# hyye/lio-mapping

Hardware: AMD Instinct MI355X
Metric: sliding-window solves/sec, 64-line 130k-pt scans, window=15 (opt_window=5) (higher is better)
Workload: dtype f64 (solve) / f32 (features); 1 GPU; HDL-64E outdoor_test_config_64, S_outdoor ray-cast scans, window_size=15 opt_window_size=5, one SolveOptimization per step, clouds resident in HBM; n_lidar_residuals=78236, local_map_points=76752, surf_stack_points=19386, parallelism=1 window

## Files before the change

lio-mapping_amd/csrc/capi.hip:

```cpp
#include <cstring>
#include <new>

#include "../../include/lio_c.h"
#include "../../include/lio_test_hooks.h"
#include "est_batch.h"
#include "seg_sort.h"
#include "estimator.h"
#include "rccl_comm.h"
#include "host_init.h"
#include "kf_batch.h"
#include <mutex>
#include <thread>
#include <atomic>

#include "mapping.h"
#include "odometry.h"
#include "pointproc.h"

using namespace lio;

struct lio_pim { std::shared_ptr<Preintegration> p; };
struct lio_est { std::unique_ptr<Estimator> e; EstConfig cfg; std::unique_ptr<MappingDev> map; lio_map_config map_cfg; std::unique_ptr<EstimatorBatch> solo; bool adopted = false; struct lio_est_batch *owner = nullptr; };
struct lio_est_batch {
  std::unique_ptr<EstimatorBatch> b, b2;
// ... 433 lines not shown
  if (!T || !out || (!corner && nc) || (!surf && ns) || (!full && nf)) return 0;
  float *o = out;
  *o++ = T->p[0]; *o++ = T->p[1]; *o++ = T->p[2]; *o++ = 0.f;
  *o++ = T->q[0]; *o++ = T->q[1]; *o++ = T->q[2]; *o++ = T->q[3];
  *o++ = float(nc); *o++ = float(ns); *o++ = float(nf); *o++ = T->q[3];
  const float *src[3] = {corner, surf, full};
  const size_t cnt[3] = {nc, ns, nf};
  for (int k = 0; k < 3; ++k) { if (cnt[k]) std::memcpy(o, src[k], cnt[k] * 4 * sizeof(float)); o += 4 * cnt[k]; }
  return size_t(o - out) / 4;
}
int lio_compact_decode(const float *d, size_t n, lio_transform_f *T, size_t *nc, size_t *ns, size_t *nf) {
  if (!d || !nc || !ns || !nf || n < 4) return LIO_ERR_ARG;
  const float lim = float(n);
  for (int k = 8; k <= 10; ++k)
    if (!(d[k] >= 0.0f && d[k] <= lim)) return LIO_ERR_ARG;
  const unsigned long long c = (unsigned long long)d[8], s = (unsigned long long)d[9], f = (unsigned long long)d[10];
  if (3ull + c + s + f != (unsigned long long)n) return LIO_ERR_ARG;
  if (T) { for (int k = 0; k < 3; ++k) T->p[k] = d[k]; for (int k = 0; k < 4; ++k) T->q[k] = d[4 + k]; }
  *nc = size_t(c); *ns = size_t(s); *nf = size_t(f);
  return LIO_OK;
}

struct Scratch {
  hipStream_t s = nullptr;
  DBuf<float4> a, b, c;
  VoxelGridDev vox;
  KnnGrid grid;
  DBuf<uint8_t> valid;
  DBuf<float4> coef;
  DBuf<float> score, tf;
  DBuf<int32_t> idx;
  DBuf<float> sqd;
  DBuf<float> bounds;
};
static Scratch &scratch() {
  static thread_local Scratch sc;
  if (!sc.s) {
    int nd = 0;
    LIO_HIP(hipGetDeviceCount(&nd));
    if (nd <= 0) throw DeviceError("no HIP device: the product has no CPU path");
    LIO_HIP(hipStreamCreate(&sc.s));
  }
  return sc;
}
static void host_bounds(const float *xyzi, size_t n, float mn[3], float mx[3]) {
  for (int d = 0; d < 3; ++d) { mn[d] = 3.4e38f; mx[d] = -3.4e38f; }
  for (size_t i = 0; i < n; ++i)
    for (int d = 0; d < 3; ++d) { float v = xyzi[4 * i + d]; if (std::isfinite(v)) { mn[d] = std::min(mn[d], v); mx[d] = std::max(mx[d], v); } }
}

int lio_voxel_grid(const float *xyzi, size_t n, float leaf, float *out, size_t *n_out) {
  if ((!xyzi && n) || !out || !n_out || !(leaf > 0)) return LIO_ERR_ARG;
  return guarded([&] {
    Scratch &sc = scratch();
    sc.a.reserve(std::max<size_t>(n, 1));
    if (n) LIO_HIP(hipMemcpyAsync(sc.a.p, xyzi, n * sizeof(float4), hipMemcpyHostToDevice, sc.s));
    size_t m = sc.vox.run(sc.a.p, n, leaf, sc.b, sc.s);
    if (m) LIO_HIP(hipMemcpyAsync(out, sc.b.p, m * sizeof(float4), hipMemcpyDeviceToHost, sc.s));
    LIO_HIP(hipStreamSynchronize(sc.s));
    *n_out = m;
    return LIO_OK;
  });
}

int lio_knn(const float *map, size_t n_map, const float *query, size_t m, int k, float radius_sq, int32_t *idx, float *sqd) {
  if ((!map && n_map) || (!query && m) || !(k == 1 || k == 5) || !idx || !sqd) return LIO_ERR_ARG;
  if (!(radius_sq > 0)) return LIO_ERR_ARG;
  return guarded([&] {
    Scratch &sc = scratch();
    sc.a.reserve(std::max<size_t>(n_map, 1)); sc.b.reserve(std::max<size_t>(m, 1));
    sc.idx.reserve(std::max<size_t>(m * k, 1)); sc.sqd.reserve(std::max<size_t>(m * k, 1));
    if (n_map) LIO_HIP(hipMemcpyAsync(sc.a.p, map, n_map * sizeof(float4), hipMemcpyHostToDevice, sc.s));
    if (m) LIO_HIP(hipMemcpyAsync(sc.b.p, query, m * sizeof(float4), hipMemcpyHostToDevice, sc.s));
    float mn[3], mx[3];
    host_bounds(map, n_map, mn, mx);
    if (n_map == 0) { mn[0] = mn[1] = mn[2] = 0; mx[0] = mx[1] = mx[2] = 0; }
    sc.grid.build(sc.a.p, n_map, mn, mx, std::sqrt(radius_sq) * 1.0001f + 1e-6f, sc.s);
    launch_knn(sc.b.p, int(m), k, radius_sq, sc.grid.sorted(), sc.grid.cells(), sc.grid.desc(), sc.idx.p, sc.sqd.p, sc.s);
    if (m) {
      LIO_HIP(hipMemcpyAsync(idx, sc.idx.p, m * k * sizeof(int32_t), hipMemcpyDeviceToHost, sc.s));
      LIO_HIP(hipMemcpyAsync(sqd, sc.sqd.p, m * k * sizeof(float), hipMemcpyDeviceToHost, sc.s));
    }
    LIO_HIP(hipStreamSynchronize(sc.s));
    return LIO_OK;
  });
}

int lio_calculate_features(const float *map, size_t n_map, const float *stack, size_t m, const lio_transform_f *T, float mm, float mp,
                           uint8_t *valid, float *coeff, float *score) {
  if ((!map && n_map) || (!stack && m) || !T || !valid || !coeff || !score || !(mm > 0)) return LIO_ERR_ARG;
  return guarded([&] {
    Scratch &sc = scratch();
    sc.a.reserve(std::max<size_t>(n_map, 1)); sc.b.reserve(std::max<size_t>(m, 1));
    sc.valid.reserve(std::max<size_t>(m, 1)); sc.coef.reserve(std::max<size_t>(m, 1)); sc.score.reserve(std::max<size_t>(m, 1)); sc.tf.reserve(8);
    if (n_map) LIO_HIP(hipMemcpyAsync(sc.a.p, map, n_map * sizeof(float4), hipMemcpyHostToDevice, sc.s));
    if (m) LIO_HIP(hipMemcpyAsync(sc.b.p, stack, m * sizeof(float4), hipMemcpyHostToDevice, sc.s));
    float tf[8] = {T->q[0], T->q[1], T->q[2], T->q[3], T->p[0], T->p[1], T->p[2], 0.f};
    LIO_HIP(hipMemcpyAsync(sc.tf.p, tf, sizeof(tf), hipMemcpyHostToDevice, sc.s));
    float mn[3], mx[3];
    host_bounds(map, n_map, mn, mx);
    if (n_map == 0) { mn[0] = mn[1] = mn[2] = 0; mx[0] = mx[1] = mx[2] = 0; }
    sc.grid.build(sc.a.p, n_map, mn, mx, std::sqrt(mm) * 1.0001f + 1e-6f, sc.s);
    FeatArgs fa{};
    fa.nframes = 1; fa.max_M = int(m); fa.min_match_sq_dis = mm; fa.min_plane_dis = mp;
    fa.fr[0].stack = sc.b.p; fa.fr[0].M = int(m); fa.fr[0].slot_off = 0; fa.fr[0].tf_index = 0;
    launch_features(fa, sc.tf.p, sc.grid.sorted(), sc.grid.cells(), sc.grid.desc(), sc.valid.p, sc.coef.p, sc.score.p, nullptr, sc.s);
    if (m) {
      LIO_HIP(hipMemcpyAsync(valid, sc.valid.p, m, hipMemcpyDeviceToHost, sc.s));
      LIO_HIP(hipMemcpyAsync(coeff, sc.coef.p, m * sizeof(float4), hipMemcpyDeviceToHost, sc.s));
      LIO_HIP(hipMemcpyAsync(score, sc.score.p, m * sizeof(float), hipMemcpyDeviceToHost, sc.s));
    }
    LIO_HIP(hipStreamSynchronize(sc.s));
    return LIO_OK;
  });
}

lio_pim *lio_pim_create(const double acc0[3], const double gyr0[3], const double ba[3], const double bg[3], double acc_n, double gyr_n,
                        double acc_w, double gyr_w, double g_norm) {
  if (!acc0 || !gyr0 || !ba || !bg) return nullptr;
  PimNoise n; n.acc_n = acc_n; n.gyr_n = gyr_n; n.acc_w = acc_w; n.gyr_w = gyr_w; n.g_norm = g_norm;
  lio_pim *h = new (std::nothrow) lio_pim;
  if (h) h->p = std::make_shared<Preintegration>(v3(acc0), v3(gyr0), v3(ba), v3(bg), n);
  return h;
}
void lio_pim_destroy(lio_pim *h) { delete h; }
int lio_pim_push_back(lio_pim *h, double dt, const double acc[3], const double gyr[3]) {
  if (!h || !acc || !gyr) return LIO_ERR_ARG;
  h->p->push_back(dt, v3(acc), v3(gyr));
  return LIO_OK;
}
int lio_pim_repropagate(lio_pim *h, const double ba[3], const double bg[3]) {
  if (!h || !ba || !bg) return LIO_ERR_ARG;
  h->p->repropagate(v3(ba), v3(bg));
  return LIO_OK;
}
int lio_pim_get(const lio_pim *h, double *sum_dt, double *dp, double *dq, double *dv, double *jac, double *cov) {
  if (!h) return LIO_ERR_ARG;
  const Preintegration &p = *h->p;
  if (sum_dt) *sum_dt = p.sum_dt;
  if (dp) { dp[0] = p.dp.x; dp[1] = p.dp.y; dp[2] = p.dp.z; }
  if (dq) { dq[0] = p.dq.x; dq[1] = p.dq.y; dq[2] = p.dq.z; dq[3] = p.dq.w; }
  if (dv) { dv[0] = p.dv.x; dv[1] = p.dv.y; dv[2] = p.dv.z; }
  if (jac) std::memcpy(jac, p.jac, sizeof(p.jac));
  if (cov) std::memcpy(cov, p.cov, sizeof(p.cov));
  return LIO_OK;
}
int lio_pim_evaluate(const lio_pim *h, const double *pi, const double *sbi, const double *pj, const double *sbj, double *res) {
  if (!h || !pi || !sbi || !pj || !sbj || !res) return LIO_ERR_ARG;
  V3d Pi, Pj; Qd Qi, Qj;
  unpack_pose(pi, Pi, Qi); unpack_pose(pj, Pj, Qj);
  h->p->evaluate(Pi, Qi, v3(sbi), v3(sbi + 3), v3(sbi + 6), Pj, Qj, v3(sbj), v3(sbj + 3), v3(sbj + 6), res);
  return LIO_OK;
}

int lio_factor_imu(const lio_pim *h, const double *pi, const double *sbi, const double *pj, const double *sbj, double *res, double *j0,
                   double *j1, double *j2, double *j3) {
  if (!h || !pi || !sbi || !pj || !sbj || !res) return LIO_ERR_ARG;
  return imu_factor(*h->p, pi, sbi, pj, sbj, res, j0, j1, j2, j3) ? LIO_OK : LIO_ERR_STATE;
}
int lio_factor_pivot_point_plane(const double point[3], const double coeff[4], const double *pp, const double *pi, const double *pex,
                                 double *res, double *j0, double *j1, double *j2) {
  if (!point || !coeff || !pp || !pi || !pex || !res) return LIO_ERR_ARG;
  ppp_factor(v3(point), coeff, pp, pi, pex, res, j0, j1, j2);
  return LIO_OK;
}
int lio_factor_prior(const double pos0[3], const double rot0[4], const double *pose, double *res, double *j) {
  if (!pos0 || !rot0 || !pose || !res) return LIO_ERR_ARG;
  prior_factor(v3(pos0), Qd(rot0[3], rot0[0], rot0[1], rot0[2]), pose, res, j);
  return LIO_OK;
}
int lio_pose_plus(const double *pose, const double *d, double *out) {
  if (!pose || !d || !out) return LIO_ERR_ARG;
  pose_plus(pose, d, out);
  return LIO_OK;
}

void lio_est_default_config(lio_est_config *c) {
  if (!c) return;
  std::memset(c, 0, sizeof(*c));
  c->window_size = 15; c->opt_window_size = 5; c->corner_filter_size = 0.2f; c->surf_filter_size = 0.4f;
  c->min_match_sq_dis = 1.0f; c->min_plane_dis = 0.2f;
  c->transform_lb.q[3] = 1.f; c->transform_lb.p[2] = -0.1f;
  c->opt_extrinsic = 0; c->imu_factor = 1; c->point_distance_factor = 0; c->prior_factor = 0; c->marginalization_factor = 1;
  c->enable_deskew = 1; c->cutoff_deskew = 0; c->keep_features = 0;
  c->acc_n = 0.1; c->gyr_n = 0.01; c->acc_w = 0.0002; c->gyr_w = 2.0e-5; c->g_norm = 9.805;
  c->max_num_iterations = 10; c->max_solver_time = 0.10; c->extrinsic_stage = 2; c->init_window_factor = 3;
}
lio_est *lio_est_create(const lio_est_config *c) {
  if (!c || c->window_size < 1 || c->opt_window_size < 1 || c->opt_window_size > c->window_size || c->window_size + 1 > LIO_MAX_FRAMES) return nullptr;
  lio_est *h = new (std::nothrow) lio_est;
  if (!h) return nullptr;
  EstConfig &e = h->cfg;
  e.W = c->window_size; e.Wo = c->opt_window_size;
  e.corner_filter_size = c->corner_filter_size; e.surf_filter_size = c->surf_filter_size;
  e.min_match_sq_dis = c->min_match_sq_dis; e.min_plane_dis = c->min_plane_dis;
// ... 402 lines not shown
}
int lio_est_batch_get_clock(const lio_est_batch *h, double *out) {
  if (!h || !out) return LIO_ERR_ARG;
  if (!h->b) return LIO_ERR_STATE;
  BatchClock c;
  const int rc = guarded([&] {
    c = const_cast<lio_est_batch *>(h)->b->clock();
    if (h->b2) {
      const BatchClock d = const_cast<lio_est_batch *>(h)->b2->clock();
      c.describe = std::max(c.describe, d.describe); c.map = std::max(c.map, d.map); c.grid_features = std::max(c.grid_features, d.grid_features);
      c.pack = std::max(c.pack, d.pack); c.solve = std::max(c.solve, d.solve); c.finish = std::max(c.finish, d.finish);
      c.fallback = std::max(c.fallback, d.fallback); c.total = std::max(c.total, d.total);
      c.n_device += d.n_device; c.n_host += d.n_host; c.rounds = std::max(c.rounds, d.rounds);
      for (int k = 0; k < 6; ++k) c.dev[k] += d.dev[k];
      c.dev_marg_wait += d.dev_marg_wait;
      for (int k = 0; k < 3; ++k) { c.kernel_ms[k] += d.kernel_ms[k]; c.kernel_launches[k] += d.kernel_launches[k]; }
    }
    return LIO_OK;
  });
  if (rc != LIO_OK) return rc;
  for (int k = 0; k < 6; ++k) out[10 + k] = c.dev[k];
  out[0] = c.describe; out[1] = c.map; out[2] = c.grid_features; out[3] = c.pack; out[4] = c.solve; out[5] = c.finish; out[6] = c.fallback; out[7] = c.total;
  out[8] = c.n_device; out[9] = c.rounds;
  out[16] = c.dev_marg_wait;
  for (int k = 0; k < 3; ++k) { out[17 + k] = c.kernel_ms[k]; out[20 + k] = double(c.kernel_launches[k]); }
  out[23] = 0.0;
  return LIO_OK;
}

int lio_est_set_factor_sharding(lio_est *h, int rank, int world, lio_allreduce_fn fn, void *user) {
  if (!h || world < 1 || rank < 0 || rank >= world) return LIO_ERR_ARG;
  h->e->shard_rank_ = rank; h->e->shard_world_ = world; h->e->allreduce_ = fn; h->e->allreduce_user_ = user;
  h->e->rccl_comm_ = nullptr;
  return LIO_OK;
}
int lio_est_set_factor_sharding_rccl(lio_est *h, lio_rccl *comm) {
  if (!h) return LIO_ERR_ARG;
  if (!comm) { h->e->rccl_comm_ = nullptr; h->e->shard_rank_ = 0; h->e->shard_world_ = 1; return LIO_OK; }
  h->e->rccl_comm_ = rccl_raw_comm(comm);
  h->e->shard_rank_ = lio_rccl_rank(comm); h->e->shard_world_ = lio_rccl_world(comm);
  h->e->allreduce_ = nullptr; h->e->allreduce_user_ = nullptr;
  return LIO_OK;
}
int lio_bench_voxel_grid(const float *xyzi, size_t n, float leaf, int reps, double *avg_ms, size_t *n_out) {
  if (!xyzi || n == 0 || !(leaf > 0) || reps < 1 || !avg_ms) return LIO_ERR_ARG;
  return guarded([&] {
    hipStream_t s = nullptr;
    LIO_HIP(hipStreamCreate(&s));
    DBuf<float4> in, out;
    in.reserve(n);
    LIO_HIP(hipMemcpyAsync(in.p, xyzi, n * sizeof(float4), hipMemcpyHostToDevice, s));
    VoxelGridDev vox;
    size_t m = 0;
    for (int w = 0; w < 2; ++w) m = vox.run(in.p, n, leaf, out, s);
    hipEvent_t e0, e1;
    LIO_HIP(hipEventCreate(&e0)); LIO_HIP(hipEventCreate(&e1));
    LIO_HIP(hipEventRecord(e0, s));
    for (int r = 0; r < reps; ++r) m = vox.run(in.p, n, leaf, out, s);
    LIO_HIP(hipEventRecord(e1, s));
    LIO_HIP(hipStreamSynchronize(s));
    float ms = 0;
    LIO_HIP(hipEventElapsedTime(&ms, e0, e1));
    *avg_ms = double(ms) / reps;
    if (n_out) *n_out = m;
    (void)hipEventDestroy(e0); (void)hipEventDestroy(e1); (void)hipStreamDestroy(s);
    return LIO_OK;
  });
}
int lio_est_bench_batched_moments(lio_est *h, int n_windows, int reps, double *avg_ms, double *bytes) {
  if (!h || n_windows < 1 || reps < 1) return LIO_ERR_ARG;
  return guarded([&] { return h->e->BenchBatchedMoments(n_windows, reps, avg_ms, bytes) ? LIO_OK : LIO_ERR_STATE; });
}
int lio_est_enable_kernel_timing(lio_est *h, int on) {
  if (!h) return LIO_ERR_ARG;
  h->e->resident_.LaunchTiming(on == -1);
  h->e->timers_.on = on > 0;
  h->e->timers_.sample = on > 1 ? on : 1;
  h->e->timers_.reset();
  return LIO_OK;
}
int lio_est_get_kernel_timing(lio_est *h, const char *name, double *total_ms, double *bytes) {
  if (total_ms) *total_ms = 0;
  if (bytes) *bytes = 0;
  if (!h || !name) return 0;
  static const char *names[KT_COUNT] = {"features", "odom_features", "odom_rows", "odom_update", "moments", "voxel", "knn_grid", "concat"};
  if (std::strcmp(name, "moments_resident") == 0) {
    int passes = 0;
    const double us = h->e->resident_.BusyUs(&passes, bytes);
    if (total_ms) *total_ms = us * 1e-3;
    return passes;
  }
  if (std::strcmp(name, "moments_resident_launch") == 0) {
    int n = 0;
    guarded([&] { n = h->e->resident_.LaunchStats(total_ms, h->e->stream()); return LIO_OK; });
    return n;
  }
  for (int k = 0; k < KT_COUNT; ++k)
    if (std::strcmp(name, names[k]) == 0) {
      const KernelTimers::Acc &a = h->e->timers_.acc[k];
      if (total_ms) *total_ms = a.ms;
      if (bytes) *bytes = a.bytes;
      return a.n;
    }
  return 0;
}

}
```

lio-mapping_amd/csrc/cloud_kernels.h:

```cpp
#pragma once
#include <cstdint>

#include "dev.h"

namespace lio {

struct VoxParams {
  float mn[3], mx[3];
  int minb[3], divb[3];
  int overflow;
  int n_valid;
};

struct Affine3f { float m[12]; };

#define LIO_MAX_FRAMES 32

struct ConcatSeg { const float4 *src; int n; int dst_off; int set_intensity; float intensity; Affine3f tf; int identity; };
struct ConcatArgs { ConcatSeg seg[LIO_MAX_FRAMES]; int nseg; int total; };
void launch_transform_concat(const ConcatArgs &a, float4 *dst, hipStream_t s);

void launch_deskew_to_end(float4 *pts, int n, const float q[4], const float p[3], float time_factor, hipStream_t s);

void launch_cloud_bounds(const float4 *pts, int n, DBuf<float> &partial, VoxParams *d_out, hipStream_t s);

class VoxelGridDev {
 public:
  size_t run(const float4 *in, size_t n, float leaf, DBuf<float4> &out, hipStream_t s, VoxParams *host_params = nullptr);
  void launch(const float4 *in, size_t n, float leaf, DBuf<float4> &out, hipStream_t s);
  size_t finish(VoxParams *host_params = nullptr);
  void set_host_signal(bool on) { use_signal_ = on; }
  VoxelGridDev() = default;
  VoxelGridDev(const VoxelGridDev &) = delete;
  VoxelGridDev &operator=(const VoxelGridDev &) = delete;

 private:
  const float4 *p_in_ = nullptr; size_t p_n_ = 0; DBuf<float4> *p_out_ = nullptr; hipStream_t p_stream_ = nullptr;
  float p_leaf_ = 0.f;
  void enqueue(bool exact);
  HostBuf<char> h_mail_;
  int *h_count_ = nullptr;
  VoxParams *h_params_ = nullptr;
  DBuf<float> partial_;
  DBuf<VoxParams> params_;
  DBuf<uint32_t> keys_, keys2_, vals_, vals2_;
  DBuf<int> count_, tile_heads_;
  DBuf<char> tmp_;
  unsigned *h_flag_ = nullptr;
  unsigned seq_ = 0;
  HostSignal sig_{};
  bool use_signal_ = true;
};

struct GridDesc {
  int origin[3];
  int dims[3];
  float inv_cell;
  int n_points;
};

class KnnGrid {
 public:
  void build(const float4 *pts, size_t n, const float mn[3], const float mx[3], float cell, hipStream_t s);
  const float4 *sorted() const { return sorted_.p; }
  const int *cells() const { return cells_.p; }
  const GridDesc &desc() const { return desc_; }

 private:
  GridDesc desc_{};
  DBuf<uint32_t> keys_, keys2_, vals_, vals2_;
  DBuf<float4> sorted_;
  DBuf<int> cells_, cnt_;
  bool cnt_dirty_ = false;
  DBuf<char> tmp_;
};

struct FeatFrame { const float4 *stack; int M; int slot_off; int tf_index; const uint32_t *order = nullptr; };
struct FeatArgs {
  FeatFrame fr[LIO_MAX_FRAMES];
  int nframes;
  int max_M;
  float min_match_sq_dis, min_plane_dis;
  int mapping_mode;
  float fixed_pz[3];
};
void launch_features(const FeatArgs &a, const float *transforms, const float4 *map_sorted, const int *cells, const GridDesc &g,
                     uint8_t *valid, float4 *coef, float *score, const int *skip_flag, hipStream_t s, float4 *abs_coef = nullptr);

void launch_knn(const float4 *query, int m, int k, float radius_sq, const float4 *map_sorted, const int *cells, const GridDesc &g,
                int32_t *idx, float *sqd, hipStream_t s);

void launch_map_round(const FeatArgs &surf, const float4 *corner_stack, int Mc, const float *transform, const float4 *corner_map,
                      const int *corner_cells, const GridDesc &corner_grid, const float4 *surf_map, const int *surf_cells,
                      const GridDesc &surf_grid, uint8_t *valid, float4 *coef, float4 *abs_coef, const int *skip_flag, hipStream_t s);

struct SolveSetup {
  float tf[LIO_MAX_FRAMES][8];
  int ntf;
  float odom_T[8];
  int set_odom;
};
struct OdomState;
void launch_solve_setup(const SolveSetup &a, float *d_transforms, OdomState *d_odom, uint8_t *valid, size_t n_valid, hipStream_t s);

struct OdomState {
  float T[8];
  int converged;
  int iters;
  int degenerate;
  int kz;
  int nsel;
};
void launch_odom_rows(const float4 *stack, int M, int nslots, const uint8_t *valid, const float4 *coef, const OdomState *st,
                      double *partials, int nblocks, hipStream_t s, int b_from_coef = 0);
void launch_odom_update(const double *partials, int nblocks, OdomState *st, int iter, hipStream_t s, int min_rows = 0, int left_update = 0,
                        OdomState *mail = nullptr, const HostSignal &sig = HostSignal());
int odom_rows_blocks(int nslots);
int odom_round_blocks(int M, int lpq);
void launch_odom_round(const FeatArgs &a, int base_slot, int round, int keep, OdomState *st, const float4 *map_sorted, const int *cells, const GridDesc &g,
                       uint8_t *valid, float4 *coef, float *score, double *partials, hipStream_t s, OdomState *mail = nullptr,
                       const HostSignal &sig = HostSignal(), int lpq = 8);

struct KfDesc {
  int slot_off, Mc, Ms;
  int map;
  int nb;
  int part_off;
  float pz[3];
};
struct KfMapDesc {
  const float4 *corner_sorted; const int *corner_cells; GridDesc corner_grid;
  const float4 *surf_sorted; const int *surf_cells; GridDesc surf_grid;
};
void launch_kf_query_keys(const KfDesc *kd, const KfMapDesc *md, const OdomState *st, int n_keyframes, int max_Mc, int max_Ms, const float4 *stack_all, uint32_t *keys,
                          hipStream_t s);
void launch_kf_round(const KfDesc *kd, const KfMapDesc *md, const OdomState *st, int n_keyframes, int max_Mc, int max_Ms, long long total_queries,
                     const float4 *stack_all, const uint32_t *order_or_null, float min_match_sq_dis, float min_plane_dis, int mapping_mode, uint8_t *valid, float4 *coef,
                     hipStream_t s);
void launch_kf_rows(const KfDesc *kd, const OdomState *st, int n_keyframes, int max_nb, const float4 *stack_all, const uint8_t *valid, const float4 *coef,
                    double *partials, int b_from_coef, hipStream_t s);
void launch_kf_update(const KfDesc *kd, OdomState *st, int n_keyframes, const double *partials, int iter, int min_rows, int left_update, int *n_converged,
                      hipStream_t s);

#if defined(__HIPCC__)
__device__ inline void reduce_partials28(const double *__restrict__ partials, int nblocks, double *ssum ) {
  __shared__ double part28[8][32];
  const int c = threadIdx.x & 31, g = threadIdx.x >> 5;
  double v = 0;
  if (c < 28 && g < 8)
    for (int b = g; b < nblocks; b += 8) v += partials[b * 28 + c];
  if (g < 8) part28[g][c] = v;
  __syncthreads();
  if (threadIdx.x < 28) {
    double s = 0;
#pragma unroll
    for (int k = 0; k < 8; ++k) s += part28[k][threadIdx.x];
    ssum[threadIdx.x] = s;
// ... 7 lines not shown
```

lio-mapping_amd/csrc/cloud_kernels.hip:

```cpp
#include <cstring>
#include <hip/hip_runtime.h>
#include <rocprim/rocprim.hpp>

#include <cfloat>
#include <climits>

#include "cloud_kernels.h"
#include "cloud_device.h"

namespace lio {

__global__ void k_transform_concat(ConcatArgs a, float4 *__restrict__ dst) {
  int gid = blockIdx.x * blockDim.x + threadIdx.x;
  if (gid >= a.total) return;
  int sidx = 0;
  for (int k = 1; k < a.nseg; ++k)
    if (gid >= a.seg[k].dst_off) sidx = k;
  const ConcatSeg &sg = a.seg[sidx];
  int local = gid - sg.dst_off;
  float4 p = sg.src[local];
  float4 o;
  if (sg.identity) {
    o = p;
  } else {
// ... 315 lines not shown
}

size_t VoxelGridDev::finish(VoxParams *host_params) {
  if (p_n_ == 0) {
    if (host_params) std::memset(host_params, 0, sizeof(*host_params));
    return 0;
  }
  const VoxMail *m = reinterpret_cast<const VoxMail *>(h_count_);
  bool redone = false;
  for (;;) {
    if (sig_.flag) wait_host_signal(sig_, p_stream_);
    else LIO_HIP(hipStreamSynchronize(p_stream_));
    if (m->range_overflow == 1 && !redone) {
      enqueue(true);
      redone = true;
      continue;
    }
    if (redone) LIO_HIP(hipStreamSynchronize(p_stream_));
    break;
  }
  int count = m->count;
  const VoxParams hp = m->params;
  if (hp.overflow) {
    p_out_->reserve(p_n_);
    LIO_HIP(hipMemcpyAsync(p_out_->p, p_in_, p_n_ * sizeof(float4), hipMemcpyDeviceToDevice, p_stream_));
    LIO_HIP(hipStreamSynchronize(p_stream_));
    count = int(p_n_);
  }
  if (host_params) *host_params = hp;
  return size_t(count);
}

size_t VoxelGridDev::run(const float4 *in, size_t n, float leaf, DBuf<float4> &out, hipStream_t s, VoxParams *host_params) {
  launch(in, n, leaf, out, s);
  return finish(host_params);
}

__global__ void k_cell_count(const float4 *__restrict__ pts, int n, GridDesc g, uint32_t *__restrict__ keys, uint32_t *__restrict__ slot,
                             int *__restrict__ cnt) {
  int i = blockIdx.x * blockDim.x + threadIdx.x;
  if (i >= n) return;
  float4 p = pts[i];
  int cx = cell_coord(p.x, g.inv_cell) - g.origin[0];
  int cy = cell_coord(p.y, g.inv_cell) - g.origin[1];
  int cz = cell_coord(p.z, g.inv_cell) - g.origin[2];
  cx = min(max(cx, 0), g.dims[0] - 1); cy = min(max(cy, 0), g.dims[1] - 1); cz = min(max(cz, 0), g.dims[2] - 1);
  const uint32_t c = uint32_t(cx + g.dims[0] * (cy + g.dims[1] * cz));
  keys[i] = c;
  slot[i] = uint32_t(atomicAdd(&cnt[c], 1));
}

__global__ void k_cell_place(const float4 *__restrict__ pts, const uint32_t *__restrict__ keys, const uint32_t *__restrict__ slot, int n,
                             const int *__restrict__ starts, float4 *__restrict__ sorted, int *__restrict__ cnt) {
  int i = blockIdx.x * blockDim.x + threadIdx.x;
  if (i >= n) return;
  float4 p = pts[i];
  p.w = __int_as_float(i);
  const uint32_t c = keys[i];
  sorted[starts[c] + int(slot[i])] = p;
  cnt[c] = 0;
}

void KnnGrid::build(const float4 *pts, size_t n, const float mn[3], const float mx[3], float cell, hipStream_t s) {
  desc_.inv_cell = 1.0f / cell;
  desc_.n_points = int(n);
  size_t ncells = 1;
  for (int d = 0; d < 3; ++d) {
    int lo = int(std::floor(mn[d] * desc_.inv_cell)) - 1;
    int hi = int(std::floor(mx[d] * desc_.inv_cell)) + 1;
    desc_.origin[d] = lo;
    desc_.dims[d] = hi - lo + 1;
    ncells *= size_t(desc_.dims[d]);
  }
  if (ncells > (size_t(1) << 30)) throw DeviceError("KnnGrid: cell table too large");
  cells_.reserve(ncells + 1);
  if (cnt_.cap < ncells + 1 || cnt_dirty_) {
    cnt_.reserve(ncells + 1);
    LIO_HIP(hipMemsetAsync(cnt_.p, 0, cnt_.cap * sizeof(int), s));
  }
  cnt_dirty_ = true;
  keys_.reserve(std::max<size_t>(n, 1)); vals_.reserve(std::max<size_t>(n, 1)); sorted_.reserve(std::max<size_t>(n, 1));
  const int ni = int(n);
  if (ni) hipLaunchKernelGGL(k_cell_count, dim3(cdiv(ni, 256)), dim3(256), 0, s, pts, ni, desc_, keys_.p, vals_.p, cnt_.p);
  size_t tmp_bytes = 0;
  LIO_HIP(rocprim::exclusive_scan(nullptr, tmp_bytes, cnt_.p, cells_.p, 0, ncells + 1, rocprim::plus<int>(), s));
  tmp_.reserve(tmp_bytes + 256);
  LIO_HIP(rocprim::exclusive_scan(tmp_.p, tmp_bytes, cnt_.p, cells_.p, 0, ncells + 1, rocprim::plus<int>(), s));
  if (ni) hipLaunchKernelGGL(k_cell_place, dim3(cdiv(ni, 256)), dim3(256), 0, s, pts, keys_.p, vals_.p, ni, cells_.p, sorted_.p, cnt_.p);
  LIO_HIP(hipGetLastError());
  cnt_dirty_ = false;
}

template <int K>
__device__ inline void knn_scan(const Vec3<float> &q, const float4 *__restrict__ map, const int *__restrict__ cells, const GridDesc &g,
                                float (&bd)[K], int (&bi)[K], int (&bj)[K]) {
#pragma unroll
  for (int k = 0; k < K; ++k) { bd[k] = INFINITY; bi[k] = INT_MAX; bj[k] = 0; }
  int cx = cell_coord(q.x, g.inv_cell) - g.origin[0];
  int cy = cell_coord(q.y, g.inv_cell) - g.origin[1];
  int cz = cell_coord(q.z, g.inv_cell) - g.origin[2];
  if (cx < 0 || cy < 0 || cz < 0 || cx >= g.dims[0] || cy >= g.dims[1] || cz >= g.dims[2]) return;
  for (int dz = -1; dz <= 1; ++dz) {
    int z = cz + dz;
    if (z < 0 || z >= g.dims[2]) continue;
    for (int dy = -1; dy <= 1; ++dy) {
      int y = cy + dy;
      if (y < 0 || y >= g.dims[1]) continue;
      int row = g.dims[0] * (y + g.dims[1] * z);
      for (int dx = -1; dx <= 1; ++dx) {
        int x = cx + dx;
        if (x < 0 || x >= g.dims[0]) continue;
        const int c0 = cells[row + x], c1 = cells[row + x + 1];
        for (int j = c0; j < c1; ++j) {
          float4 p = map[j];
          float ddx = p.x - q.x, ddy = p.y - q.y, ddz = p.z - q.z;
          float d = ddx * ddx;
          d += ddy * ddy;
          d += ddz * ddz;
          int idx = __float_as_int(p.w);
          if (d < bd[K - 1] || (d == bd[K - 1] && idx < bi[K - 1])) {
            bd[K - 1] = d; bi[K - 1] = idx; bj[K - 1] = j;
#pragma unroll
            for (int k = K - 1; k > 0; --k) {
              bool sw = bd[k - 1] > bd[k] || (bd[k - 1] == bd[k] && bi[k - 1] > bi[k]);
              float td = sw ? bd[k - 1] : bd[k];
              int ti = sw ? bi[k - 1] : bi[k];
              int tj = sw ? bj[k - 1] : bj[k];
              bd[k - 1] = sw ? bd[k] : bd[k - 1];
              bi[k - 1] = sw ? bi[k] : bi[k - 1];
              bj[k - 1] = sw ? bj[k] : bj[k - 1];
              bd[k] = td; bi[k] = ti; bj[k] = tj;
            }
          }
        }
      }
    }
  }
}

template <int K>
__global__ void k_knn(const float4 *__restrict__ query, int m, float radius_sq, const float4 *__restrict__ map,
                      const int *__restrict__ cells, GridDesc g, int32_t *__restrict__ idx, float *__restrict__ sqd, int kout) {
  int i = blockIdx.x * blockDim.x + threadIdx.x;
  if (i >= m) return;
  float4 q4 = query[i];
  float bd[K]; int bi[K], bj[K];
  knn_scan<K>(Vec3<float>(q4.x, q4.y, q4.z), map, cells, g, bd, bi, bj);
  for (int k = 0; k < kout; ++k) {
    bool ok = bi[k] != INT_MAX && bd[k] < radius_sq;
    idx[i * kout + k] = ok ? bi[k] : -1;
    sqd[i * kout + k] = ok ? bd[k] : INFINITY;
  }
}

void launch_knn(const float4 *query, int m, int k, float radius_sq, const float4 *map_sorted, const int *cells, const GridDesc &g,
                int32_t *idx, float *sqd, hipStream_t s) {
  if (m <= 0) return;
  if (k == 1) hipLaunchKernelGGL(k_knn<1>, dim3(cdiv(m, 128)), dim3(128), 0, s, query, m, radius_sq, map_sorted, cells, g, idx, sqd, k);
  else hipLaunchKernelGGL(k_knn<5>, dim3(cdiv(m, 128)), dim3(128), 0, s, query, m, radius_sq, map_sorted, cells, g, idx, sqd, k);
  LIO_HIP(hipGetLastError());
}

template <bool MAPPING, int LPQ>
__global__ void __launch_bounds__(FEAT_THREADS) k_features(FeatArgs a, const float *__restrict__ transforms, const float4 *__restrict__ map,
                                                          const int *__restrict__ cells, GridDesc g, uint8_t *__restrict__ valid,
                                                          float4 *__restrict__ coef, float *__restrict__ score, const int *__restrict__ skip_flag,
                                                          float4 *__restrict__ abs_coef) {
  if (skip_flag && *skip_flag) return;
  features_block<MAPPING, LPQ>(a.fr[blockIdx.y], feat_scalars(a), int(blockIdx.x), transforms, map, cells, g, valid, coef, score, abs_coef);
}
// ... 339 lines not shown
```

lio-mapping_amd/csrc/estimator.hip:

```cpp
#include "estimator.h"
#include "est_batch.h"
#include "marg_kernels.h"
#include "rccl_comm.h"

#include <atomic>
#include <cfloat>
#include <climits>
#include <cstring>

namespace lio {

static const bool g_debug_timing = std::getenv("LIO_DEBUG_TIMING") != nullptr;

static V3d R2ypr(const M3d &R) {
  V3d n(R(0, 0), R(1, 0), R(2, 0)), o(R(0, 1), R(1, 1), R(2, 1)), a(R(0, 2), R(1, 2), R(2, 2));
  double y = atan2(n.y, n.x);
  double p = atan2(-n.z, n.x * cos(y) + n.y * sin(y));
  double r = atan2(a.x * sin(y) - a.y * cos(y), -o.x * sin(y) + o.y * cos(y));
  return V3d(y, p, r) / M_PI * 180.0;
}
static M3d ypr2R(const V3d &ypr) {
  double y = ypr.x / 180.0 * M_PI, p = ypr.y / 180.0 * M_PI, r = ypr.z / 180.0 * M_PI;
  M3d Rz, Ry, Rx;
  Rz(0, 0) = cos(y); Rz(0, 1) = -sin(y); Rz(1, 0) = sin(y); Rz(1, 1) = cos(y); Rz(2, 2) = 1;
// ... 438 lines not shown
  }
  std::memcpy(su.odom_T, &tfs[size_t(W_) * 8], 8 * sizeof(float));
  su.set_odom = cfg_.imu_factor ? 1 : 0;
  d_transforms_.reserve(tfs.size());
  launch_solve_setup(su, d_transforms_.p, d_odom_.p, f_valid_.p, total_slots_, stream_);
  FeatArgs fa{};
  fa.min_match_sq_dis = cfg_.min_match_sq_dis; fa.min_plane_dis = cfg_.min_plane_dis;
  const int last_static = cfg_.imu_factor ? W_ - 1 : W_;
  for (int i = pivot + 1; i <= last_static; ++i) {
    FeatFrame &f = fa.fr[fa.nframes++];
    f.stack = stacks_[i].buf.p; f.M = int(stacks_[i].n); f.slot_off = slot_off_[i]; f.tf_index = i;
    fa.max_M = std::max(fa.max_M, f.M);
  }
  {
    double mq = 0;
    for (int k = 0; k < fa.nframes; ++k) mq += fa.fr[k].M;
    hipStream_t sf = cfg_.imu_factor ? stream2_ : stream_;
    if (sf != stream_) {
      LIO_HIP(hipEventRecord(ev_fork_, stream_));
      LIO_HIP(hipStreamWaitEvent(sf, ev_fork_, 0));
    }
    th = timers_.begin(KT_FEATURES, 16.0 * (mq + double(local_filtered_.n)) + 40.0 * mq + 32.0 * mq, sf);
    launch_features(fa, d_transforms_.p, grid_.sorted(), grid_.cells(), grid_.desc(), f_valid_.p, f_coef_.p, f_score_.p, nullptr, sf);
    timers_.end(th, sf);
    if (sf != stream_) LIO_HIP(hipEventRecord(ev_join_, sf));
  }
  laser_odom_iters_ = 0; laser_odom_kz_ = 0;
  if (cfg_.imu_factor) {
    OdomState st{};
    bool have_state = false;
    std::memcpy(st.T, &tfs[size_t(W_) * 8], 8 * sizeof(float));
    const int M = int(stacks_[W_].n);
    const bool mail = host_signal_ && !timers_.on;
    HostSignal sig{};
    if (M > 0) {
      const int lpq = 8;
      const int nb = odom_round_blocks(M, lpq);
      d_odom_partials_.reserve(size_t(nb) * 28);
      FeatArgs fo{};
      fo.min_match_sq_dis = cfg_.min_match_sq_dis; fo.min_plane_dis = cfg_.min_plane_dis;
      fo.nframes = 1; fo.max_M = M;
      fo.fr[0].stack = stacks_[W_].buf.p; fo.fr[0].M = M; fo.fr[0].tf_index = 0; fo.fr[0].slot_off = slot_off_[W_];
      const int chunk_end[4] = {3, 5, 7, 10};
      int chunk = 0;
      for (int iter = 0; iter < 10; ++iter) {
        if (iter == chunk_end[chunk]) {
          if (mail) {
            wait_host_signal(sig, stream_);
          } else {
            LIO_HIP(hipMemcpyAsync(h_odom_.p, d_odom_.p, sizeof(st), hipMemcpyDeviceToHost, stream_));
            LIO_HIP(hipStreamSynchronize(stream_));
          }
          st = *h_odom_.p;
          if (st.converged) { have_state = true; break; }
          ++chunk;
        }
        if (mail) { sig.flag = h_signal_.p + 128; sig.seq = ++signal_seq_[1]; }
        const double ns = keep_mult > 1 ? double(iter + 1) * M : double(M);
        int t1h = timers_.begin(KT_ODOM_FEATURES, 16.0 * (double(M) + double(local_filtered_.n)) + 72.0 * M + 33.0 * ns, stream_);
        launch_odom_round(fo, slot_off_[W_], iter, keep_mult > 1 ? 1 : 0, d_odom_.p, grid_.sorted(), grid_.cells(), grid_.desc(), f_valid_.p, f_coef_.p,
                          f_score_.p, d_odom_partials_.p, stream_, mail ? h_odom_.p : nullptr, sig, lpq);
        timers_.end(t1h, stream_);
      }
    }
    LIO_HIP(hipStreamWaitEvent(stream_, ev_join_, 0));
    if (!have_state) {
      if (sig.flag) {
        wait_host_signal(sig, stream_);
      } else {
        LIO_HIP(hipMemcpyAsync(h_odom_.p, d_odom_.p, sizeof(st), hipMemcpyDeviceToHost, stream_));
        LIO_HIP(hipStreamSynchronize(stream_));
      }
      st = *h_odom_.p;
      timers_.resolve();
    }
    laser_odom_iters_ = st.iters;
    laser_odom_kz_ = st.degenerate ? st.kz : 0;
    laser_odom_transform_ = Rigidf(Quat<float>(st.T[3], st.T[0], st.T[1], st.T[2]), Vec3<float>(st.T[4], st.T[5], st.T[6]));
    if (keep_mult > 1) nslots_[W_] = int(stacks_[W_].n) * std::max(1, st.iters);
  } else {
    LIO_HIP(hipStreamSynchronize(stream_));
    timers_.resolve();
  }
  const double t2 = now_ms();
  if (rep) {
    rep->ms_build_map = t1 - t0; rep->ms_features = t2 - t1; rep->n_local_map = int(local_filtered_.n);
    rep->laser_odom_iterations = laser_odom_iters_; rep->laser_odom_kz = laser_odom_kz_;
  }
}

void Estimator::VectorToParams(WindowParams &P) const {
  const int pivot = W_ - Wo_;
  P.Wo = Wo_;
  P.pose.resize(Wo_ + 1); P.sb.resize(Wo_ + 1);
  for (int i = 0, oi = pivot; i <= Wo_; ++i, ++oi) {
    Qd q = fromRot(Rs_[oi]);
    P.pose[i] = {Ps_[oi].x, Ps_[oi].y, Ps_[oi].z, q.x, q.y, q.z, q.w};
    P.sb[i] = {Vs_[oi].x, Vs_[oi].y, Vs_[oi].z, Bas_[oi].x, Bas_[oi].y, Bas_[oi].z, Bgs_[oi].x, Bgs_[oi].y, Bgs_[oi].z};
  }
  P.ex = {transform_lb_.pos.x, transform_lb_.pos.y, transform_lb_.pos.z, transform_lb_.rot.x, transform_lb_.rot.y, transform_lb_.rot.z,
          transform_lb_.rot.w};
}

void Estimator::ParamsToVector(const WindowParams &P) {
  const int pivot = W_ - Wo_;
  const V3d origin_P0 = Ps_[pivot];
  const V3d origin_R0 = R2ypr(Rs_[pivot]);
  const M3d R00 = toRot(normalized(Qd(P.pose[0][6], P.pose[0][3], P.pose[0][4], P.pose[0][5])));
  const V3d origin_R00 = R2ypr(R00);
  const double y_diff = origin_R0.x - origin_R00.x;
  M3d rot_diff = ypr2R(V3d(y_diff, 0, 0));
  if (std::fabs(std::fabs(origin_R0.y) - 90) < 1.0 || std::fabs(std::fabs(origin_R00.y) - 90) < 1.0) rot_diff = Rs_[pivot] * transpose(R00);
  {
    Rigidd trans_pivot(fromRot(Rs_[pivot]), Ps_[pivot]);
    Rigidd trans_opt_pivot(fromRot(rot_diff * R00), origin_P0);
    for (int idx = 0; idx < pivot; ++idx) {
      Rigidd trans_idx(fromRot(Rs_[idx]), Ps_[idx]);
      Rigidd t = compose(compose(trans_opt_pivot, rinverse(trans_pivot)), trans_idx);
      Ps_[idx] = t.pos;
      Rs_[idx] = toRot(normalized(t.rot));
    }
  }
  for (int i = 0, oi = pivot; i <= Wo_; ++i, ++oi) {
    Qd qi(P.pose[i][6], P.pose[i][3], P.pose[i][4], P.pose[i][5]);
    Rs_[oi] = rot_diff * toRot(normalized(qi));
    Ps_[oi] = rot_diff * V3d(P.pose[i][0] - P.pose[0][0], P.pose[i][1] - P.pose[0][1], P.pose[i][2] - P.pose[0][2]) + origin_P0;
    Vs_[oi] = rot_diff * V3d(P.sb[i][0], P.sb[i][1], P.sb[i][2]);
    Bas_[oi] = V3d(P.sb[i][3], P.sb[i][4], P.sb[i][5]);
    Bgs_[oi] = V3d(P.sb[i][6], P.sb[i][7], P.sb[i][8]);
  }
  transform_lb_.pos = Vec3<float>(float(P.ex[0]), float(P.ex[1]), float(P.ex[2]));
  transform_lb_.rot = Quat<float>(float(P.ex[6]), float(P.ex[3]), float(P.ex[4]), float(P.ex[5]));
}

void Estimator::LidarEval(const WindowParams &P, std::vector<FrameMoments> &m) {
  LidarLaunch(P);
  LidarWait(m);
}

void Estimator::FillMomentArgs(MomentArgs &ma, int &max_slots) const {
  const int pivot = W_ - Wo_;
  ma = MomentArgs{};
  max_slots = 0;
  for (int i = 1; i <= Wo_; ++i) {
    MomentFrame &f = ma.fr[ma.nframes++];
    const int idx = pivot + i;
    f.stack = stacks_[idx].buf.p; f.M = std::max<int>(1, int(stacks_[idx].n)); f.slot_off = slot_off_[idx]; f.nslots = nslots_[idx];
    f.slot_begin = 0; f.slot_end = f.nslots;
    if (Sharded()) {
      f.slot_begin = int((long long)f.nslots * shard_rank_ / shard_world_);
      f.slot_end = int((long long)f.nslots * (shard_rank_ + 1) / shard_world_);
    }
    max_slots = std::max(max_slots, f.nslots);
  }
  ma.blocks_per_frame = moment_blocks_per_frame(max_slots);
  const int rb = resident_.Bpf(max_slots, ma.nframes);
  if (rb > 0) ma.blocks_per_frame = rb;
}

void Estimator::LidarLaunch(const WindowParams &P) {
  MomentArgs ma;
  int max_slots = 0;
  FillMomentArgs(ma, max_slots);
  for (int i = 1; i <= Wo_; ++i) relative_lidar_pose(P.pose[0].data(), P.pose[i].data(), P.ex.data(), ma.fr[i - 1].R, ma.fr[i - 1].t);
  LidarLaunchMoments(ma);
}
// ... 485 lines not shown
```

Measured before the change: 2158 solves/s.

## Replace rocprim cell-table scan with single-pass decoupled-lookback chained scan

The k-NN grid build's exclusive scan over cell counts moves from rocprim's two-call exclusive_scan to a custom single-pass kernel. The new kernel takes tiles by ticket and uses decoupled lookback through tagged 64-bit state words, so there is one launch and no separate temporary-storage sizing. A watchdog timeout writes a failure code to coherent host memory, and check() after each synchronize throws if the scan gave up. This cuts launch and scan overhead per grid build, at the cost of spin-wait risk, a custom correctness burden and extra host status checks.

```diff
diff --git a/lio-mapping_amd/csrc/capi.hip b/lio-mapping_amd/csrc/capi.hip
--- a/lio-mapping_amd/csrc/capi.hip
+++ b/lio-mapping_amd/csrc/capi.hip
@@ -539,6 +539,7 @@
       LIO_HIP(hipMemcpyAsync(sqd, sc.sqd.p, m * k * sizeof(float), hipMemcpyDeviceToHost, sc.s));
     }
     LIO_HIP(hipStreamSynchronize(sc.s));
+    sc.grid.check();
     return LIO_OK;
   });
 }
@@ -568,6 +569,7 @@
       LIO_HIP(hipMemcpyAsync(score, sc.score.p, m * sizeof(float), hipMemcpyDeviceToHost, sc.s));
     }
     LIO_HIP(hipStreamSynchronize(sc.s));
+    sc.grid.check();
     return LIO_OK;
   });
 }
@@ -1136,7 +1138,9 @@
 int lio_est_get_kernel_timing(lio_est *h, const char *name, double *total_ms, double *bytes) {
   if (total_ms) *total_ms = 0;
   if (bytes) *bytes = 0;
-  if (!h || !name) return 0;
+  if (!name) return 0;
+  if (std::strcmp(name, "sort_fallbacks") == 0) return int(chained_fallbacks());
+  if (!h) return 0;
   static const char *names[KT_COUNT] = {"features", "odom_features", "odom_rows", "odom_update", "moments", "voxel", "knn_grid", "concat"};
   if (std::strcmp(name, "moments_resident") == 0) {
     int passes = 0;
diff --git a/lio-mapping_amd/csrc/chain_scan.h b/lio-mapping_amd/csrc/chain_scan.h
--- /dev/null
+++ b/lio-mapping_amd/csrc/chain_scan.h
@@ -0,0 +1,25 @@
+#pragma once
+#include <cstdint>
+
+#include "dev.h"
+
+namespace lio {
+
+long long chained_fallbacks();
+
+class ChainScan {
+ public:
+  void enqueue(const int *in, int *out, size_t n, hipStream_t s);
+  void check();
+  ChainScan() = default;
+  ChainScan(const ChainScan &) = delete;
+  ChainScan &operator=(const ChainScan &) = delete;
+
+ private:
+  DBuf<uint32_t> ws_;
+  HostBuf<unsigned> h_status_;
+  int cap_tiles_ = 0;
+  uint32_t seq_ = 0, ticket_base_ = 0;
+};
+
+}
diff --git a/lio-mapping_amd/csrc/chain_scan.hip b/lio-mapping_amd/csrc/chain_scan.hip
--- /dev/null
+++ b/lio-mapping_amd/csrc/chain_scan.hip
@@ -0,0 +1,169 @@
+#include <hip/hip_runtime.h>
+
+#include <algorithm>
+#include <atomic>
+
+#include "chain_scan.h"
+
+namespace lio {
+
+using gran_t = unsigned long long;
+#define CH_AGG 1u
+#define CH_INC 2u
+#define CH_WAIT_TICKS 20000000ll
+#define CH_CODE_WAIT 1u
+#define CH_CODE_TICKET 2u
+
+__device__ __forceinline__ gran_t ch_load(const gran_t *p) { return __hip_atomic_load(p, __ATOMIC_RELAXED, __HIP_MEMORY_SCOPE_AGENT); }
+__device__ __forceinline__ void ch_store(gran_t *p, uint32_t tag, uint32_t v) {
+  __hip_atomic_store(p, (gran_t(tag) << 32) | gran_t(v), __ATOMIC_RELAXED, __HIP_MEMORY_SCOPE_AGENT);
+}
+__device__ __forceinline__ uint32_t ch_status(const uint32_t *status) { return __hip_atomic_load(status, __ATOMIC_RELAXED, __HIP_MEMORY_SCOPE_AGENT); }
+__device__ __forceinline__ void ch_give_up(uint32_t *status, unsigned *h_status, uint32_t code) {
+  __hip_atomic_store(status, code, __ATOMIC_RELAXED, __HIP_MEMORY_SCOPE_AGENT);
+  host_store(h_status, unsigned(code));
+}
+__device__ __forceinline__ bool ch_stalled(long long t0, uint32_t *status, unsigned *h_status) {
+  if (ch_status(status) != 0u) return true;
+  if (wall_clock64() - t0 > CH_WAIT_TICKS) { ch_give_up(status, h_status, CH_CODE_WAIT); return true; }
+  __builtin_amdgcn_s_sleep(1);
+  return false;
+}
+
+static std::atomic<long long> g_fallbacks{0};
+long long chained_fallbacks() { return g_fallbacks.load(); }
+
+#define CS_THREADS 1024
+#define CS_ROWS 4
+constexpr int CS_NW = CS_THREADS / 64, CS_ROW = CS_THREADS * 4, CS_TILE = CS_ROW * CS_ROWS;
+static_assert(CS_NW * CS_ROWS == 64, "one wave scans the (row, wave) sums");
+#define CS_WS_STATUS 1
+#define CS_WS_GRAN 16
+
+__global__ void __launch_bounds__(CS_THREADS) k_chain_scan(const int *__restrict__ in, int *__restrict__ out, int n, int ntiles, gran_t *state, uint32_t *ticket,
+                                                           uint32_t ticket_base, uint32_t seq, uint32_t *status, unsigned *h_status) {
+  __shared__ uint32_t part[64];
+  __shared__ uint32_t s_excl;
+  __shared__ int s_tile, s_fail;
+  const int tid = threadIdx.x, lane = tid & 63, wave = tid >> 6;
+  if (tid == 0) {
+    s_tile = int(atomicAdd(ticket, 1u) - ticket_base);
+    s_fail = ch_status(status) != 0u;
+  }
+  __syncthreads();
+  const int tile = s_tile;
+  if (tile < 0 || tile >= ntiles) {
+    if (tid == 0) ch_give_up(status, h_status, CH_CODE_TICKET);
+    return;
+  }
+  int4 v[CS_ROWS];
+  uint32_t incl[CS_ROWS], own[CS_ROWS];
+  if (!s_fail) {
+#pragma unroll
+    for (int r = 0; r < CS_ROWS; ++r) {
+      const int i = tile * CS_TILE + r * CS_ROW + tid * 4;
+      if (i + 3 < n) v[r] = *reinterpret_cast<const int4 *>(in + i);
+      else { v[r].x = i < n ? in[i] : 0; v[r].y = i + 1 < n ? in[i + 1] : 0; v[r].z = i + 2 < n ? in[i + 2] : 0; v[r].w = 0; }
+    }
+#pragma unroll
+    for (int r = 0; r < CS_ROWS; ++r) {
+      own[r] = uint32_t(v[r].x) + uint32_t(v[r].y) + uint32_t(v[r].z) + uint32_t(v[r].w);
+      uint32_t x = own[r];
+#pragma unroll
+      for (int o = 1; o < 64; o <<= 1) { const uint32_t t = __shfl_up(x, o, 64); if (lane >= o) x += t; }
+      incl[r] = x;
+      if (lane == 63) part[r * CS_NW + wave] = x;
+    }
+  }
+  __syncthreads();
+  if (wave == 0) {
+    const uint32_t tag = seq << 2;
+    uint32_t excl = 0;
+    bool fail = s_fail != 0;
+    if (!fail) {
+      const uint32_t p = part[lane];
+      uint32_t x = p;
+#pragma unroll
+      for (int o = 1; o < 64; o <<= 1) { const uint32_t t = __shfl_up(x, o, 64); if (lane >= o) x += t; }
+      part[lane] = x - p;
+      const uint32_t total = __shfl(x, 63, 64);
+      if (lane == 0 && tile > 0) ch_store(state + tile, tag | CH_AGG, total);
+      int j = tile - 1;
+      const long long t0 = wall_clock64();
+      for (;;) {
+        const int jj = j - lane;
+        const gran_t g = jj >= 0 ? ch_load(state + jj) : (gran_t(tag | CH_INC) << 32);
+        const uint32_t gt = uint32_t(g >> 32);
+        const unsigned long long b_inc = __ballot(gt == (tag | CH_INC)), b_not = __ballot(gt != (tag | CH_INC) && gt != (tag | CH_AGG));
+        const int first_inc = b_inc ? __builtin_ctzll(b_inc) : 64, first_not = b_not ? __builtin_ctzll(b_not) : 64;
+        const int take = first_inc < first_not ? first_inc + 1 : first_not;
+        uint32_t a = lane < take ? uint32_t(g) : 0u;
+#pragma unroll
+        for (int o = 32; o > 0; o >>= 1) a += __shfl_xor(a, o, 64);
+        excl += a;
+        if (first_inc < first_not) break;
+        j -= take;
+        if (first_not < 64 && __any(ch_stalled(t0, status, h_status))) { fail = true; break; }
+      }
+      if (lane == 0) {
+        if (!fail) ch_store(state + tile, tag | CH_INC, excl + total);
+        s_excl = excl;
+      }
+    }
+    if (lane == 0 && fail) s_fail = 1;
+  }
+  __syncthreads();
+  const bool fail = s_fail != 0;
+#pragma unroll
+  for (int r = 0; r < CS_ROWS; ++r) {
+    const int i = tile * CS_TILE + r * CS_ROW + tid * 4;
+    int4 o;
+    if (fail) { o.x = o.y = o.z = o.w = 0; }
+    else {
+      const uint32_t b = s_excl + part[r * CS_NW + wave] + (incl[r] - own[r]);
+      o.x = int(b); o.y = int(b + uint32_t(v[r].x)); o.z = int(uint32_t(o.y) + uint32_t(v[r].y)); o.w = int(uint32_t(o.z) + uint32_t(v[r].z));
+    }
+    if (i + 3 < n) *reinterpret_cast<int4 *>(out + i) = o;
+    else {
+      if (i < n) out[i] = o.x;
+      if (i + 1 < n) out[i + 1] = o.y;
+      if (i + 2 < n) out[i + 2] = o.z;
+    }
+  }
+}
+
+void ChainScan::enqueue(const int *in, int *out, size_t n, hipStream_t s) {
+  if (n == 0) return;
+  if (n > (size_t(1) << 30) + 1) throw DeviceError("ChainScan: table too large");
+  const int ni = int(n), ntiles = cdiv(ni, CS_TILE);
+  if (!h_status_.p) h_status_.alloc(16, hipHostMallocCoherent, true);
+  if (ntiles > cap_tiles_ || !ws_.p) {
+    const int cap = std::max(ntiles + ntiles / 2, 256);
+    ws_.reserve(size_t(CS_WS_GRAN) + size_t(cap) * 2, s);
+    LIO_HIP(hipMemsetAsync(ws_.p, 0, ws_.cap * sizeof(uint32_t), s));
+    cap_tiles_ = cap; ticket_base_ = 0;
+  }
+  if (++seq_ >= (1u << 30)) {
+    LIO_HIP(hipMemsetAsync(ws_.p, 0, ws_.cap * sizeof(uint32_t), s));
+    seq_ = 1; ticket_base_ = 0;
+  }
+  hipLaunchKernelGGL(k_chain_scan, dim3(ntiles), dim3(CS_THREADS), 0, s, in, out, ni, ntiles, reinterpret_cast<gran_t *>(ws_.p + CS_WS_GRAN), ws_.p, ticket_base_, seq_,
+                     ws_.p + CS_WS_STATUS, h_status_.p);
+  LIO_HIP(hipGetLastError());
+  ticket_base_ += uint32_t(ntiles);
+}
+
+void ChainScan::check() {
+  if (!h_status_.p || __atomic_load_n(h_status_.p, __ATOMIC_ACQUIRE) == 0) return;
+  const unsigned code = *h_status_.p;
+  g_fallbacks.fetch_add(1);
+  __atomic_store_n(h_status_.p, 0u, __ATOMIC_RELEASE);
+  if (ws_.p) {
+    LIO_HIP(hipDeviceSynchronize());
+    LIO_HIP(hipMemset(ws_.p, 0, ws_.cap * sizeof(uint32_t)));
+    ticket_base_ = 0;
+  }
+  throw DeviceError("K-NN grid: the cell table's scan gave up waiting (code " + std::to_string(code) + ")");
+}
+
+}
diff --git a/lio-mapping_amd/csrc/cloud_kernels.h b/lio-mapping_amd/csrc/cloud_kernels.h
--- a/lio-mapping_amd/csrc/cloud_kernels.h
+++ b/lio-mapping_amd/csrc/cloud_kernels.h
@@ -2,6 +2,7 @@
 #include <cstdint>
 
 #include "dev.h"
+#include "chain_scan.h"
 
 namespace lio {
 
@@ -65,6 +66,7 @@
   const float4 *sorted() const { return sorted_.p; }
   const int *cells() const { return cells_.p; }
   const GridDesc &desc() const { return desc_; }
+  void check() { scan_.check(); }
 
  private:
   GridDesc desc_{};
@@ -72,7 +74,7 @@
   DBuf<float4> sorted_;
   DBuf<int> cells_, cnt_;
   bool cnt_dirty_ = false;
-  DBuf<char> tmp_;
+  ChainScan scan_;
 };
 
 struct FeatFrame { const float4 *stack; int M; int slot_off; int tf_index; const uint32_t *order = nullptr; };
diff --git a/lio-mapping_amd/csrc/cloud_kernels.hip b/lio-mapping_amd/csrc/cloud_kernels.hip
--- a/lio-mapping_amd/csrc/cloud_kernels.hip
+++ b/lio-mapping_amd/csrc/cloud_kernels.hip
@@ -421,10 +421,7 @@
   keys_.reserve(std::max<size_t>(n, 1)); vals_.reserve(std::max<size_t>(n, 1)); sorted_.reserve(std::max<size_t>(n, 1));
   const int ni = int(n);
   if (ni) hipLaunchKernelGGL(k_cell_count, dim3(cdiv(ni, 256)), dim3(256), 0, s, pts, ni, desc_, keys_.p, vals_.p, cnt_.p);
-  size_t tmp_bytes = 0;
-  LIO_HIP(rocprim::exclusive_scan(nullptr, tmp_bytes, cnt_.p, cells_.p, 0, ncells + 1, rocprim::plus<int>(), s));
-  tmp_.reserve(tmp_bytes + 256);
-  LIO_HIP(rocprim::exclusive_scan(tmp_.p, tmp_bytes, cnt_.p, cells_.p, 0, ncells + 1, rocprim::plus<int>(), s));
+  scan_.enqueue(cnt_.p, cells_.p, ncells + 1, s);
   if (ni) hipLaunchKernelGGL(k_cell_place, dim3(cdiv(ni, 256)), dim3(256), 0, s, pts, keys_.p, vals_.p, ni, cells_.p, sorted_.p, cnt_.p);
   LIO_HIP(hipGetLastError());
   cnt_dirty_ = false;
diff --git a/lio-mapping_amd/csrc/estimator.hip b/lio-mapping_amd/csrc/estimator.hip
--- a/lio-mapping_amd/csrc/estimator.hip
+++ b/lio-mapping_amd/csrc/estimator.hip
@@ -544,6 +544,7 @@
     LIO_HIP(hipStreamSynchronize(stream_));
     timers_.resolve();
   }
+  grid_.check();
   const double t2 = now_ms();
   if (rep) {
     rep->ms_build_map = t1 - t0; rep->ms_features = t2 - t1; rep->n_local_map = int(local_filtered_.n);
```

Measured after the change: 2179 solves/s, median of 4. Within noise of the previous version (+1.0%).
